# JBanks/GraphGym

Measured on AMD Instinct MI355X. Metric: aggregated edges/sec + achieved HBM GB/s, GCN d=256 on 100M-edge scale-free, higher is better.
Workload: dtype f32

## Files before the change

### graphgym_amd/csrc/gemm.hip

```cpp
#include "common.h"
#include "vecio.h"
#include "bf16x3.h"
#include <limits.h>

namespace mp {

constexpr int BM = 128, BN = 128, BK = 16;

constexpr int kPlaneBytes = 16 * 256;
__device__ __forceinline__ int swz_off(int row, int ch) {
  return 256 * row + 16 * (ch ^ (((row & 3) << 2) | ((row >> 2) & 3)));
}
__device__ __forceinline__ bf16x8 tr_read8(const unsigned char* plane, int col0, int lane) {
  const int g = lane >> 4, q = (lane & 15) >> 2, p = lane & 3;
  const int chunk = ((col0 + 16 * (g & 1)) >> 3) + (p >> 1);
  const int r0 = 8 * (g >> 1) + q;
  typedef __attribute__((address_space(3))) s16x4 lds_s16x4;
  const s16x4 lo = __builtin_amdgcn_ds_read_tr16_b64_v4i16(
      (lds_s16x4*)(plane + swz_off(r0, chunk) + 8 * (p & 1)));
  const s16x4 hi = __builtin_amdgcn_ds_read_tr16_b64_v4i16(
      (lds_s16x4*)(plane + swz_off(r0 + 4, chunk) + 8 * (p & 1)));
  const s16x8 v = {lo[0], lo[1], lo[2], lo[3], hi[0], hi[1], hi[2], hi[3]};
  return __builtin_bit_cast(bf16x8, v);
}
#define MP_STASH8(IMG, AT, lo, hi)                                                                      \
  do {                                                                                                  \
    bf16x8 s_[3];                                                                                       \
    const float v_[8] = {lo[0], lo[1], lo[2], lo[3], hi[0], hi[1], hi[2], hi[3]};                       \
    split3_bf16(v_, s_[0], s_[1], s_[2]);                                                               \
    _Pragma("unroll") for (int pl_ = 0; pl_ < 3; ++pl_) *reinterpret_cast<bf16x8*>(&IMG[pl_] AT) = s_[pl_]; \
  } while (0)
#define MP_ZERO_ACC(acc, NI, NJ)                         \
  _Pragma("unroll") for (int i_ = 0; i_ < (NI); ++i_)    \
  _Pragma("unroll") for (int j_ = 0; j_ < (NJ); ++j_)    \
  _Pragma("unroll") for (int r_ = 0; r_ < 16; ++r_) acc[i_][j_][r_] = 0.f

template <bool DUAL, bool VEC>
__global__ __launch_bounds__(kBlock, 3) void dense_fused_kernel(const float* __restrict__ P, int64_t ldp,
                                                                const float* __restrict__ W,
                                                                const float* __restrict__ Q, int64_t ldq,
                                                                const float* __restrict__ Wid,
                                                                const float* __restrict__ bias, int act,
                                                                float* __restrict__ out, int64_t ldo, int64_t M,
                                                                int32_t F, int32_t d) {
  __shared__ __attribute__((aligned(16))) unsigned char Aimg[2][3][BM * 32];
  __shared__ __attribute__((aligned(16))) unsigned char Bimg[2][3][kPlaneBytes];
  const int tid = threadIdx.x;
  const int lane = tid & 63;
  const int wave = tid >> 6;
  const int wm = wave >> 1, wn = wave & 1;
  const int ncb = (d + BN - 1) / BN;
  const int64_t m0 = (int64_t)(blockIdx.x / ncb) * BM;
  const int n0 = (int)(blockIdx.x % ncb) * BN;

  const int a_row = tid >> 1;
  const int a_k = (tid & 1) * 8;
  const int b_k = tid >> 4;
  const int b_n = (tid & 15) * 8;
  const int64_t g_row = m0 + a_row;
  const bool row_ok = g_row < M;
  const int KT = DUAL ? 2 * F : F;

  f32x4 ra[2], rb[2];
  auto fetch = [&](int kt) {
    const f32x4 z = {0.f, 0.f, 0.f, 0.f};
    const int k = kt + a_k;
    const int kb = kt + b_k;
    if constexpr (VEC) {
      const bool second = DUAL && k >= F;
      const float* src = second ? Q + g_row * ldq + (k - F) : P + g_row * ldp + k;
      const bool ok = row_ok && k < KT;
      ra[0] = ok ? *reinterpret_cast<const f32x4*>(src) : z;
      ra[1] = ok ? *reinterpret_cast<const f32x4*>(src + 4) : z;
      const bool second_b = DUAL && kb >= F;
      const float* wsrc = (second_b ? Wid + (int64_t)(kb - F) * d : W + (int64_t)kb * d) + n0 + b_n;
#pragma unroll
      for (int q = 0; q < 2; ++q)
        rb[q] = (kb < KT && n0 + b_n + 4 * q < d) ? *reinterpret_cast<const f32x4*>(wsrc + 4 * q) : z;
    } else {
#pragma unroll
      for (int i = 0; i < 8; ++i) {
        const int ki = k + i;
        float v = 0.f;
        if (row_ok && ki < KT) v = (DUAL && ki >= F) ? Q[g_row * ldq + (ki - F)] : P[g_row * ldp + ki];
        ra[i >> 2][i & 3] = v;
      }
      const bool second_b = DUAL && kb >= F;
      const float* wrow = second_b ? Wid + (int64_t)(kb - F) * d : W + (int64_t)kb * d;
#pragma unroll
      for (int q = 0; q < 2; ++q)
#pragma unroll
        for (int i = 0; i < 4; ++i) {
          const int nn = n0 + b_n + 4 * q + i;
          rb[q][i] = (kb < KT && nn < d) ? wrow[nn] : 0.f;
        }
    }
  };
  auto stash = [&](int buf) {
    MP_STASH8(Aimg[buf], [a_row * 32 + (a_k >> 3) * 16], ra[0], ra[1]);
    MP_STASH8(Bimg[buf], [swz_off(b_k, b_n >> 3)], rb[0], rb[1]);
  };

  f32x16 acc[2][2];
  MP_ZERO_ACC(acc, 2, 2);

  fetch(0);
  stash(0);
  __syncthreads();
  const int ntiles = (KT + BK - 1) / BK;
  const int fr = lane & 31, fk = lane >> 5;
  for (int t = 0; t < ntiles; ++t) {
    const int buf = t & 1;
    if (t + 1 < ntiles) fetch((t + 1) * BK);
    {
      bf16x8 as[2][3], bs3[2][3];
#pragma unroll
      for (int i = 0; i < 2; ++i)
#pragma unroll
        for (int pl = 0; pl < 3; ++pl)
          as[i][pl] = *reinterpret_cast<const bf16x8*>(&Aimg[buf][pl][(wm * 64 + i * 32 + fr) * 32 + fk * 16]);
#pragma unroll
      for (int j = 0; j < 2; ++j)
#pragma unroll
        for (int pl = 0; pl < 3; ++pl) bs3[j][pl] = tr_read8(Bimg[buf][pl], wn * 64 + j * 32, lane);
#pragma unroll
      for (int i = 0; i < 2; ++i)
#pragma unroll
        for (int j = 0; j < 2; ++j) mfma6(acc[i][j], as[i], bs3[j]);
    }
    if (t + 1 < ntiles) stash(buf ^ 1);
    __syncthreads();
  }

#pragma unroll
  for (int j = 0; j < 2; ++j) {
    const int col = n0 + wn * 64 + j * 32 + fr;
    const bool col_ok = col < d;
    const float bv = (bias != nullptr && col_ok) ? bias[col] : 0.f;
#pragma unroll
    for (int i = 0; i < 2; ++i) {
#pragma unroll
      for (int r = 0; r < 16; ++r) {
        const int64_t row = m0 + wm * 64 + i * 32 + (r & 3) + 8 * (r >> 2) + 4 * fk;
        float v = acc[i][j][r] + bv;
        if (act == MP_ACT_RELU) v = fmaxf(v, 0.f);
        if (col_ok && row < M) out[row * ldo + col] = v;
      }
    }
  }
}


struct ChunkRows { int64_t mb, me; };
__device__ __forceinline__ ChunkRows chunk_rows(int64_t c, int64_t chunk, int64_t M) {
  const int64_t mb = c * chunk;
  return {mb, mb + chunk < M ? mb + chunk : M};
}

template <bool VEC, bool RELU>
__global__ __launch_bounds__(kBlock, 3) void dense_wgrad_kernel(const float* __restrict__ P, int64_t ldp,
                                                                const float* G, int64_t ldg,
                                                                const float* __restrict__ Y, int64_t ldy,
                                                                float* GM, int64_t ldgm,
                                                                int64_t M, int32_t F, int32_t d, int64_t chunk,
                                                                float* __restrict__ slabs,
                                                                float* __restrict__ bias_slabs) {
  constexpr int BT = 128;
  __shared__ __attribute__((aligned(16))) unsigned char Pimg[2][3][kPlaneBytes];
  __shared__ __attribute__((aligned(16))) unsigned char Gimg[2][3][kPlaneBytes];
  const int tid = threadIdx.x, lane = tid & 63, wave = tid >> 6;
  const int wm = wave >> 1, wn = wave & 1;
  const int tf = (F + BT - 1) / BT, td = (d + BT - 1) / BT;
  const int tile = blockIdx.x % (tf * td);
  const int64_t c = blockIdx.x / (tf * td);
  const int f0 = (tile / td) * BT, d0 = (tile % td) * BT;
  const ChunkRows cr = chunk_rows(c, chunk, M);
  const int64_t mb = cr.mb, me = cr.me;

  const int l_row = tid >> 4;
  const int l_col = (tid & 15) * 8;
  f32x4 rp[2], rg[2];
  const f32x4 z = {0.f, 0.f, 0.f, 0.f};
  auto fetch = [&](int64_t m0) {
    const int64_t m = m0 + l_row;
    const bool ok = m < me;
    const float* ps = P + m * ldp + f0 + l_col;
    const float* gs = G + m * ldg + d0 + l_col;
    if constexpr (VEC) {
      rp[0] = (ok && f0 + l_col < F) ? *reinterpret_cast<const f32x4*>(ps) : z;
      rp[1] = (ok && f0 + l_col + 4 < F) ? *reinterpret_cast<const f32x4*>(ps + 4) : z;
      rg[0] = (ok && d0 + l_col < d) ? *reinterpret_cast<const f32x4*>(gs) : z;
      rg[1] = (ok && d0 + l_col + 4 < d) ? *reinterpret_cast<const f32x4*>(gs + 4) : z;
      if constexpr (RELU) {
        const float* ys = Y + m * ldy + d0 + l_col;
        const f32x4 y0 = (ok && d0 + l_col < d) ? *reinterpret_cast<const f32x4*>(ys) : z;
        const f32x4 y1 = (ok && d0 + l_col + 4 < d) ? *reinterpret_cast<const f32x4*>(ys + 4) : z;
#pragma unroll
        for (int i = 0; i < 4; ++i) {
          rg[0][i] = y0[i] > 0.f ? rg[0][i] : 0.f;
          rg[1][i] = y1[i] > 0.f ? rg[1][i] : 0.f;
        }
        if (GM != nullptr && f0 == 0 && ok) {
          float* go = GM + m * ldgm + d0 + l_col;
          if (d0 + l_col < d) *reinterpret_cast<f32x4*>(go) = rg[0];
          if (d0 + l_col + 4 < d) *reinterpret_cast<f32x4*>(go + 4) = rg[1];
        }
      }
    } else {
#pragma unroll
      for (int i = 0; i < 8; ++i) {
        rp[i >> 2][i & 3] = (ok && f0 + l_col + i < F) ? ps[i] : 0.f;
        float gv = (ok && d0 + l_col + i < d) ? gs[i] : 0.f;
        if constexpr (RELU) {
          const bool in = ok && d0 + l_col + i < d;
          const float yv = in ? Y[m * ldy + d0 + l_col + i] : 0.f;
          gv = yv > 0.f ? gv : 0.f;
          if (GM != nullptr && f0 == 0 && in) GM[m * ldgm + d0 + l_col + i] = gv;
        }
        rg[i >> 2][i & 3] = gv;
      }
    }
  };
  auto stash = [&](int buf) {
    const float pv[8] = {rp[0][0], rp[0][1], rp[0][2], rp[0][3], rp[1][0], rp[1][1], rp[1][2], rp[1][3]};
    const float gv[8] = {rg[0][0], rg[0][1], rg[0][2], rg[0][3], rg[1][0], rg[1][1], rg[1][2], rg[1][3]};
    bf16x8 sp[3], sg[3];
    split3_bf16(pv, sp[0], sp[1], sp[2]);
    split3_bf16(gv, sg[0], sg[1], sg[2]);
    const int off = swz_off(l_row, l_col >> 3);
#pragma unroll
    for (int pl = 0; pl < 3; ++pl) {
      *reinterpret_cast<bf16x8*>(&Pimg[buf][pl][off]) = sp[pl];
      *reinterpret_cast<bf16x8*>(&Gimg[buf][pl][off]) = sg[pl];
    }
  };
  f32x16 acc[2][2];
  MP_ZERO_ACC(acc, 2, 2);

  const bool do_bias = bias_slabs != nullptr && f0 == 0;
  float bs[8];
#pragma unroll
  for (int i = 0; i < 8; ++i) bs[i] = 0.f;
  auto tally = [&]() {
#pragma unroll
    for (int i = 0; i < 4; ++i) { bs[i] += rg[0][i]; bs[4 + i] += rg[1][i]; }
  };

  const int fr = lane & 31, fk = lane >> 5;
  const int64_t ntiles = (me - mb + BK - 1) / BK;
  if (ntiles > 0) {
    fetch(mb);
    if (do_bias) tally();
    stash(0);
  }
  __syncthreads();
  for (int64_t t = 0; t < ntiles; ++t) {
    const int buf = (int)(t & 1);
    if (t + 1 < ntiles) {
      fetch(mb + (t + 1) * BK);
      if (do_bias) tally();
    }
    {
      bf16x8 as[2][3], bs3[2][3];
#pragma unroll
      for (int i = 0; i < 2; ++i)
#pragma unroll
        for (int pl = 0; pl < 3; ++pl) {
          as[i][pl] = tr_read8(Pimg[buf][pl], wm * 64 + i * 32, lane);
          bs3[i][pl] = tr_read8(Gimg[buf][pl], wn * 64 + i * 32, lane);
        }
#pragma unroll
      for (int i = 0; i < 2; ++i)
#pragma unroll
        for (int j = 0; j < 2; ++j) mfma6(acc[i][j], as[i], bs3[j]);
    }
    if (t + 1 < ntiles) stash(buf ^ 1);
    __syncthreads();
  }
  float* slab = slabs + c * (int64_t)F * d;
#pragma unroll
  for (int j = 0; j < 2; ++j) {
    const int col = d0 + wn * 64 + j * 32 + fr;
#pragma unroll
    for (int i = 0; i < 2; ++i) {
#pragma unroll
      for (int r = 0; r < 16; ++r) {
        const int row = f0 + wm * 64 + i * 32 + (r & 3) + 8 * (r >> 2) + 4 * fk;
        if (row < F && col < d) slab[(int64_t)row * d + col] = acc[i][j][r];
      }
    }
  }
  if (do_bias) {
    float (*red)[BT] = reinterpret_cast<float (*)[BT]>(&Pimg[0][0][0]);
    *reinterpret_cast<f32x4*>(&red[l_row][l_col]) = f32x4{bs[0], bs[1], bs[2], bs[3]};
    *reinterpret_cast<f32x4*>(&red[l_row][l_col + 4]) = f32x4{bs[4], bs[5], bs[6], bs[7]};
    __syncthreads();
    if (tid < BT && d0 + tid < d) {
      float sacc = 0.f;
#pragma unroll
      for (int r = 0; r < BK; ++r) sacc += red[r][tid];
      bias_slabs[c * (int64_t)d + d0 + tid] = sacc;
    }
  }
}

template <bool RELU>
__global__ __launch_bounds__(kBlock, 2) void dense_wgrad_wide_kernel(const float* __restrict__ P, int64_t ldp,
                                                                     const float* G, int64_t ldg,
                                                                     const float* __restrict__ Y, int64_t ldy,
                                                                     float* GM, int64_t ldgm,
                                                                     int64_t M, int32_t F, int32_t d, int64_t chunk,
                                                                     float* __restrict__ slabs,
                                                                     float* __restrict__ bias_slabs) {
  constexpr int BF = 256, BD = 128;
  __shared__ __attribute__((aligned(16))) unsigned char Pimg[2][3][2][kPlaneBytes];
  __shared__ __attribute__((aligned(16))) unsigned char Gimg[2][3][kPlaneBytes];
  const int tid = threadIdx.x, lane = tid & 63, wave = tid >> 6;
  const int tf = (F + BF - 1) / BF, td = (d + BD - 1) / BD;
  const int tile = blockIdx.x % (tf * td);
  const int64_t c = blockIdx.x / (tf * td);
  const int f0 = (tile / td) * BF, d0 = (tile % td) * BD;
  const ChunkRows cr = chunk_rows(c, chunk, M);
  const int64_t mb = cr.mb, me = cr.me;

  const int l_row = tid >> 4;
  const int l_col = (tid & 15) * 8;
  f32x4 rp[2][2], rg[2];
  const f32x4 z = {0.f, 0.f, 0.f, 0.f};
  auto fetch = [&](int64_t m0) {
    const int64_t m = m0 + l_row;
    const bool ok = m < me;
    const float* gs = G + m * ldg + d0 + l_col;
#pragma unroll
    for (int h = 0; h < 2; ++h) {
      const int fc = f0 + 128 * h + l_col;
      const float* ps = P + m * ldp + fc;
      rp[h][0] = (ok && fc < F) ? *reinterpret_cast<const f32x4*>(ps) : z;
      rp[h][1] = (ok && fc + 4 < F) ? *reinterpret_cast<const f32x4*>(ps + 4) : z;
    }
    rg[0] = (ok && d0 + l_col < d) ? *reinterpret_cast<const f32x4*>(gs) : z;
    rg[1] = (ok && d0 + l_col + 4 < d) ? *reinterpret_cast<const f32x4*>(gs + 4) : z;
    if constexpr (RELU) {
      const float* ys = Y + m * ldy + d0 + l_col;
      const f32x4 y0 = (ok && d0 + l_col < d) ? *reinterpret_cast<const f32x4*>(ys) : z;
      const f32x4 y1 = (ok && d0 + l_col + 4 < d) ? *reinterpret_cast<const f32x4*>(ys + 4) : z;
#pragma unroll
      for (int i = 0; i < 4; ++i) {
        rg[0][i] = y0[i] > 0.f ? rg[0][i] : 0.f;
        rg[1][i] = y1[i] > 0.f ? rg[1][i] : 0.f;
      }
      if (GM != nullptr && f0 == 0 && ok) {
        float* go = GM + m * ldgm + d0 + l_col;
        if (d0 + l_col < d) *reinterpret_cast<f32x4*>(go) = rg[0];
        if (d0 + l_col + 4 < d) *reinterpret_cast<f32x4*>(go + 4) = rg[1];
      }
    }
  };
  auto stash = [&](int buf) {
    const int off = swz_off(l_row, l_col >> 3);
#pragma unroll
    for (int h = 0; h < 2; ++h) {
      MP_STASH8(Pimg[buf], [h][off], rp[h][0], rp[h][1]);
    }
    MP_STASH8(Gimg[buf], [off], rg[0], rg[1]);
  };
  f32x16 acc[2][4];
  MP_ZERO_ACC(acc, 2, 4);

  const bool do_bias = bias_slabs != nullptr && f0 == 0;
  float bs[8];
#pragma unroll
  for (int i = 0; i < 8; ++i) bs[i] = 0.f;
  auto tally = [&]() {
#pragma unroll
    for (int i = 0; i < 4; ++i) { bs[i] += rg[0][i]; bs[4 + i] += rg[1][i]; }
  };

  const int fr = lane & 31, fk = lane >> 5;
  const int64_t ntiles = (me - mb + BK - 1) / BK;
  if (ntiles > 0) {
    fetch(mb);
    if (do_bias) tally();
    stash(0);
  }
  __syncthreads();
  for (int64_t t = 0; t < ntiles; ++t) {
    const int buf = (int)(t & 1);
    if (t + 1 < ntiles) {
      fetch(mb + (t + 1) * BK);
      if (do_bias) tally();
    }
    {
      bf16x8 as[2][3];
#pragma unroll
      for (int i = 0; i < 2; ++i)
#pragma unroll
        for (int pl = 0; pl < 3; ++pl) as[i][pl] = tr_read8(Pimg[buf][pl][wave >> 1], (wave & 1) * 64 + i * 32, lane);
#pragma unroll
      for (int j = 0; j < 4; ++j) {
        bf16x8 b3[3];
#pragma unroll
        for (int pl = 0; pl < 3; ++pl) b3[pl] = tr_read8(Gimg[buf][pl], j * 32, lane);
#pragma unroll
        for (int i = 0; i < 2; ++i) mfma6(acc[i][j], as[i], b3);
      }
    }
    if (t + 1 < ntiles) stash(buf ^ 1);
    __syncthreads();
  }
  float* slab = slabs + c * (int64_t)F * d;
#pragma unroll
  for (int j = 0; j < 4; ++j) {
    const int col = d0 + j * 32 + fr;
#pragma unroll
    for (int i = 0; i < 2; ++i) {
#pragma unroll
      for (int r = 0; r < 16; ++r) {
        const int row = f0 + wave * 64 + i * 32 + (r & 3) + 8 * (r >> 2) + 4 * fk;
        if (row < F && col < d) slab[(int64_t)row * d + col] = acc[i][j][r];
      }
    }
  }
  if (do_bias) {
    float (*red)[BD] = reinterpret_cast<float (*)[BD]>(&Pimg[0][0][0][0]);
    *reinterpret_cast<f32x4*>(&red[l_row][l_col]) = f32x4{bs[0], bs[1], bs[2], bs[3]};
    *reinterpret_cast<f32x4*>(&red[l_row][l_col + 4]) = f32x4{bs[4], bs[5], bs[6], bs[7]};
    __syncthreads();
    if (tid < BD && d0 + tid < d) {
      float sacc = 0.f;
#pragma unroll
      for (int r = 0; r < BK; ++r) sacc += red[r][tid];
      bias_slabs[c * (int64_t)d + d0 + tid] = sacc;
    }
  }
}

constexpr int WPC_MFMA_WAVES = 8, WPC_LOAD_WAVES = 4;
constexpr int WPC_THREADS = 64 * (WPC_MFMA_WAVES + WPC_LOAD_WAVES);

template <bool RELU, int DT>
__global__ __launch_bounds__(WPC_THREADS, 3) void dense_wgrad_pc_kernel(const float* __restrict__ P, int64_t ldp,
                                                                        const float* G, int64_t ldg,
                                                                        const float* __restrict__ Y, int64_t ldy,
                                                                        float* GM, int64_t ldgm, int64_t M, int32_t F,
                                                                        int32_t d, int64_t chunk,
                                                                        float* __restrict__ slabs,
                                                                        float* __restrict__ bias_slabs) {
  __shared__ __attribute__((aligned(16))) unsigned char Pimg[2][3][2][kPlaneBytes];
  __shared__ __attribute__((aligned(16))) unsigned char Gimg[2][3][DT][kPlaneBytes];
  const int tid = threadIdx.x, lane = tid & 63;
  const int wave = __builtin_amdgcn_readfirstlane(tid >> 6);
  const int tf = (F + 255) / 256, td = (d + 128 * DT - 1) / (128 * DT);
  const int tile = (int)(blockIdx.x % (unsigned)(tf * td));
  const int64_t c = blockIdx.x / (unsigned)(tf * td);
  const int f0 = (tile / td) * 256, d0 = (tile % td) * 128 * DT;
  const ChunkRows cr = chunk_rows(c, chunk, M);
  const int64_t mb = cr.mb, me = cr.me;
  const int64_t ntiles = (me - mb + BK - 1) / BK;

  constexpr int NSET = RELU ? 2 : 3;
  const int64_t nsteps = (ntiles + NSET - 1) / NSET * NSET;
  if (wave >= WPC_MFMA_WAVES) {
    const int lt = tid - 64 * WPC_MFMA_WAVES;
    const int l_row = lt >> 4;
    const int l_col = (lt & 15) * 8;
    const bool do_bias = bias_slabs != nullptr && f0 == 0;
    float bs[2][8];
#pragma unroll
    for (int h = 0; h < 2; ++h)
#pragma unroll
      for (int i = 0; i < 8; ++i) bs[h][i] = 0.f;
    bool pin[2], gin[2];
    int pcol[2], gcol[2];
#pragma unroll
    for (int h = 0; h < 2; ++h) {
      const int fc = 128 * h + l_col;
      pin[h] = f0 + fc < F; gin[h] = d0 + fc < d;
      pcol[h] = pin[h] ? f0 + fc : 0; gcol[h] = gin[h] ? d0 + fc : 0;
    }
    f32x4 rp[NSET][2][2], rg[NSET][2][2], ry[RELU ? NSET : 1][2][2];
    auto fetch = [&](int s, int64_t tile) {
      int64_t m = mb + tile * BK + l_row;
      m = m < me ? m : me - 1;
#pragma unroll
      for (int h = 0; h < 2; ++h) {
        const float* ps = P + m * ldp + pcol[h];
        rp[s][h][0] = *reinterpret_cast<const f32x4*>(ps);
        rp[s][h][1] = *reinterpret_cast<const f32x4*>(ps + 4);
        if (h < DT) {
          const float* gs = G + m * ldg + gcol[h];
          rg[s][h][0] = *reinterpret_cast<const f32x4*>(gs);
          rg[s][h][1] = *reinterpret_cast<const f32x4*>(gs + 4);
          if constexpr (RELU) {
            const float* ys = Y + m * ldy + gcol[h];
            ry[s][h][0] = *reinterpret_cast<const f32x4*>(ys);
            ry[s][h][1] = *reinterpret_cast<const f32x4*>(ys + 4);
          }
        }
      }
    };
    auto stash = [&](int s, int64_t tile, int buf) {
      const int off = swz_off(l_row, l_col >> 3);
      const int64_t m = mb + tile * BK + l_row;
      const bool ok = m < me;
#pragma unroll
      for (int h = 0; h < 2; ++h) {
        float pv[8];
#pragma unroll
        for (int i = 0; i < 8; ++i) pv[i] = (ok && pin[h]) ? rp[s][h][i >> 2][i & 3] : 0.f;
        bf16x8 sp[3];
        split3_bf16(pv, sp[0], sp[1], sp[2]);
#pragma unroll
        for (int pl = 0; pl < 3; ++pl) *reinterpret_cast<bf16x8*>(&Pimg[buf][pl][h][off]) = sp[pl];
        if (h < DT) {
          float gv[8];
#pragma unroll
          for (int i = 0; i < 8; ++i) {
            gv[i] = (ok && gin[h]) ? rg[s][h][i >> 2][i & 3] : 0.f;
            if constexpr (RELU) gv[i] = ry[s][h][i >> 2][i & 3] > 0.f ? gv[i] : 0.f;
          }
          if constexpr (RELU) {
            if (GM != nullptr && f0 == 0 && ok && gin[h]) {
              float* go = GM + m * ldgm + gcol[h];
              *reinterpret_cast<f32x4*>(go) = f32x4{gv[0], gv[1], gv[2], gv[3]};
              *reinterpret_cast<f32x4*>(go + 4) = f32x4{gv[4], gv[5], gv[6], gv[7]};
            }
          }
          bf16x8 sg[3];
          split3_bf16(gv, sg[0], sg[1], sg[2]);
#pragma unroll
          for (int pl = 0; pl < 3; ++pl) *reinterpret_cast<bf16x8*>(&Gimg[buf][pl][h][off]) = sg[pl];
          if (do_bias) {
#pragma unroll
            for (int i = 0; i < 8; ++i) bs[h][i] += gv[i];
          }
        }
      }
    };
#pragma unroll
    for (int k = 0; k < NSET; ++k) fetch(k, k);
    stash(0, 0, 0);
    fetch(0, NSET);
    role_barrier();
    for (int64_t base = 0; base < nsteps; base += NSET) {
#pragma unroll
      for (int u = 0; u < NSET; ++u) {
        const int64_t t = base + u;
        const int sidx = (u + 1) % NSET;
        stash(sidx, t + 1, (int)((t + 1) & 1));
        fetch(sidx, t + 1 + NSET);
        role_barrier();
      }
    }
    if (do_bias) {
      float (*red)[256] = reinterpret_cast<float (*)[256]>(&Pimg[0][0][0][0]);
#pragma unroll
      for (int h = 0; h < DT; ++h) {
        *reinterpret_cast<f32x4*>(&red[l_row][128 * h + l_col]) = f32x4{bs[h][0], bs[h][1], bs[h][2], bs[h][3]};
        *reinterpret_cast<f32x4*>(&red[l_row][128 * h + l_col + 4]) = f32x4{bs[h][4], bs[h][5], bs[h][6], bs[h][7]};
      }
    }
    role_barrier();
    if (do_bias && lt < 128 * DT && d0 + lt < d) {
      const float (*red)[256] = reinterpret_cast<const float (*)[256]>(&Pimg[0][0][0][0]);
      float sacc = 0.f;
#pragma unroll
      for (int r = 0; r < BK; ++r) sacc += red[r][lt];
      bias_slabs[c * (int64_t)d + d0 + lt] = sacc;
    }
  } else {
    constexpr int NI = DT;
    const int wf = DT == 2 ? wave >> 1 : wave;
    const int wd = DT == 2 ? wave & 1 : 0;
    const int f_lo = DT == 2 ? wf * 64 : wf * 32;
    const int fr = lane & 31, fk = lane >> 5;
    f32x16 acc[NI][4];
    MP_ZERO_ACC(acc, NI, 4);
    role_barrier();
    for (int64_t t = 0; t < nsteps; ++t) {
      const int buf = (int)(t & 1);
#pragma unroll
      for (int i = 0; i < NI; ++i) {
        bf16x8 as[3];
#pragma unroll
        for (int pl = 0; pl < 3; ++pl) as[pl] = tr_read8(Pimg[buf][pl][f_lo >> 7], (f_lo & 127) + i * 32, lane);
#pragma unroll
        for (int j = 0; j < 4; ++j) {
          bf16x8 b3[3];
#pragma unroll
          for (int pl = 0; pl < 3; ++pl) b3[pl] = tr_read8(Gimg[buf][pl][wd], j * 32, lane);
          mfma6(acc[i][j], as, b3);
          __builtin_amdgcn_sched_barrier(0);
        }
      }
      role_barrier();
    }
    role_barrier();
    float* slab = slabs + c * (int64_t)F * d;
#pragma unroll
    for (int j = 0; j < 4; ++j) {
      const int col = d0 + wd * 128 + j * 32 + fr;
#pragma unroll
      for (int i = 0; i < NI; ++i) {
#pragma unroll
        for (int r = 0; r < 16; ++r) {
          const int row = f0 + f_lo + i * 32 + (r & 3) + 8 * (r >> 2) + 4 * fk;
          if (row < F && col < d) slab[(int64_t)row * d + col] = acc[i][j][r];
        }
      }
    }
  }
}

template <bool RELU>
__global__ __launch_bounds__(kBlock) void narrow_wgrad_kernel(const float* __restrict__ P, int64_t ldp,
                                                              const float* G, int64_t ldg,
                                                              const float* __restrict__ Y, int64_t ldy, float* GM,
                                                              int64_t ldgm, int64_t M, int32_t F, int32_t d,
                                                              int64_t chunk, float* __restrict__ slabs,
                                                              float* __restrict__ bias_slabs) {
  const int c = blockIdx.y * kBlock + threadIdx.x;
  const int64_t ch = blockIdx.x;
  const ChunkRows cr = chunk_rows(ch, chunk, M);
  const int64_t mb = cr.mb, me = cr.me;
  if (c >= d) return;
  float acc[8];
#pragma unroll
  for (int f = 0; f < 8; ++f) acc[f] = 0.f;
  float bs = 0.f;
  constexpr int UR = 4;
  for (int64_t m0 = mb; m0 < me; m0 += UR) {
    float gv[UR];
#pragma unroll
    for (int u = 0; u < UR; ++u) {
      const int64_t m = m0 + u;
      float v = 0.f;
      if (m < me) {
        v = G[m * ldg + c];
        if constexpr (RELU) {
          v = Y[m * ldy + c] > 0.f ? v : 0.f;
          if (GM != nullptr) GM[m * ldgm + c] = v;
        }
      }
      gv[u] = v;
    }
#pragma unroll
    for (int u = 0; u < UR; ++u) {
      const int64_t m = m0 + u;
      if (m < me) {
        bs += gv[u];
        const float* pr = P + m * ldp;
#pragma unroll
        for (int f = 0; f < 8; ++f)
          if (f < F) acc[f] = fmaf(pr[f], gv[u], acc[f]);
      }
    }
  }
  float* slab = slabs + ch * (int64_t)F * d;
  for (int f = 0; f < F; ++f) slab[(int64_t)f * d + c] = acc[f];
  if (bias_slabs != nullptr) bias_slabs[ch * (int64_t)d + c] = bs;
}

template <bool RELU, int FT>
__global__ __launch_bounds__(kBlock) void narrow_wgrad_vec_kernel(const float* __restrict__ P, int64_t ldp,
                                                                  const float* G, int64_t ldg,
                                                                  const float* __restrict__ Y, int64_t ldy, float* GM,
                                                                  int64_t ldgm, int64_t M, int32_t F, int32_t d,
                                                                  int64_t chunk, float* __restrict__ slabs,
                                                                  float* __restrict__ bias_slabs) {
  __shared__ __attribute__((aligned(16))) float red[kBlock * 4 * (FT + 1)];
  const int ncg = d >> 2;
  const int nrl = kBlock / ncg;
  const int cg = threadIdx.x % ncg, rl = threadIdx.x / ncg;
  const int64_t ch = blockIdx.x;
  const ChunkRows cr = chunk_rows(ch, chunk, M);
  const int64_t mb = cr.mb, me = cr.me;
  f32x4 acc[FT];
#pragma unroll
  for (int f = 0; f < FT; ++f) acc[f] = f32x4{0.f, 0.f, 0.f, 0.f};
  f32x4 bs = {0.f, 0.f, 0.f, 0.f};
  constexpr int UR = FT == 1 ? 8 : 4;
  for (int64_t m0 = mb + rl; m0 < me; m0 += (int64_t)UR * nrl) {
    f32x4 gv[UR], yv[UR];
    float pv[UR][FT];
#pragma unroll
    for (int u = 0; u < UR; ++u) {
      int64_t m = m0 + (int64_t)u * nrl;
      m = m < me ? m : me - 1;
      gv[u] = *reinterpret_cast<const f32x4*>(G + m * ldg + 4 * cg);
      if constexpr (RELU) yv[u] = *reinterpret_cast<const f32x4*>(Y + m * ldy + 4 * cg);
      const float* pr = P + m * ldp;
#pragma unroll
      for (int f = 0; f < FT; ++f) pv[u][f] = pr[f < F ? f : F - 1];
    }
#pragma unroll
    for (int u = 0; u < UR; ++u) {
      const int64_t m = m0 + (int64_t)u * nrl;
      if (m < me) {
        f32x4 v = gv[u];
        if constexpr (RELU) {
          v[0] = yv[u][0] > 0.f ? v[0] : 0.f; v[1] = yv[u][1] > 0.f ? v[1] : 0.f;
          v[2] = yv[u][2] > 0.f ? v[2] : 0.f; v[3] = yv[u][3] > 0.f ? v[3] : 0.f;
          if (GM != nullptr) *reinterpret_cast<f32x4*>(GM + m * ldgm + 4 * cg) = v;
        }
        bs += v;
#pragma unroll
        for (int f = 0; f < FT; ++f) acc[f] += pv[u][f] * v;
      }
    }
  }
#pragma unroll
  for (int f = 0; f < FT; ++f) *reinterpret_cast<f32x4*>(&red[((rl * (FT + 1) + f) * ncg + cg) * 4]) = acc[f];
  *reinterpret_cast<f32x4*>(&red[((rl * (FT + 1) + FT) * ncg + cg) * 4]) = bs;
  __syncthreads();
  if (rl == 0) {
    float* slab = slabs + ch * (int64_t)F * d;
    for (int f = 0; f <= FT; ++f) {
      if (f < F || (f == FT && bias_slabs != nullptr)) {
        f32x4 t = {0.f, 0.f, 0.f, 0.f};
        for (int r = 0; r < nrl; ++r) t += *reinterpret_cast<const f32x4*>(&red[((r * (FT + 1) + f) * ncg + cg) * 4]);
        if (f < FT) *reinterpret_cast<f32x4*>(slab + (int64_t)f * d + 4 * cg) = t;
        else *reinterpret_cast<f32x4*>(bias_slabs + ch * (int64_t)d + 4 * cg) = t;
      }
    }
  }
}

__global__ __launch_bounds__(kBlock) void narrow_out_wgrad_kernel(const float* __restrict__ P, int64_t ldp,
                                                                  const float* __restrict__ G, int64_t ldg, int64_t M,
                                                                  int32_t F, int32_t d, int64_t chunk,
                                                                  float* __restrict__ slabs,
                                                                  float* __restrict__ bias_slabs) {
  __shared__ float red[64][4][17];
  const int ncg = F >> 2;
  const int64_t ch = blockIdx.x;
  const ChunkRows cr = chunk_rows(ch, chunk, M);
  const int64_t mb = cr.mb, me = cr.me;
  float* slab = slabs + ch * (int64_t)F * d;
  for (int cg0 = 0; cg0 < ncg; cg0 += 64) {
    const int ng = ncg - cg0 < 64 ? ncg - cg0 : 64;
    const int nrl = kBlock / 64;
    const int cgi = threadIdx.x & 63, rl = threadIdx.x >> 6;
    const bool on = cgi < ng;
    const int f0 = 4 * (cg0 + cgi);
    float acc[4][16];
#pragma unroll
    for (int f = 0; f < 4; ++f)
#pragma unroll
      for (int j = 0; j < 16; ++j) acc[f][j] = 0.f;
    float bs[16];
#pragma unroll
    for (int j = 0; j < 16; ++j) bs[j] = 0.f;
    constexpr int UR = 4;
    for (int64_t m0 = mb + rl; m0 < me; m0 += (int64_t)UR * nrl) {
      f32x4 pv[UR];
      float gv[UR][16];
#pragma unroll
      for (int u = 0; u < UR; ++u) {
        int64_t m = m0 + (int64_t)u * nrl;
        m = m < me ? m : me - 1;
        pv[u] = on ? *reinterpret_cast<const f32x4*>(P + m * ldp + f0) : f32x4{0.f, 0.f, 0.f, 0.f};
#pragma unroll
        for (int j = 0; j < 16; ++j) gv[u][j] = G[m * ldg + (j < d ? j : d - 1)];
      }
#pragma unroll
      for (int u = 0; u < UR; ++u) {
        if (m0 + (int64_t)u * nrl < me) {
#pragma unroll
          for (int j = 0; j < 16; ++j) {
            bs[j] += gv[u][j];
#pragma unroll
            for (int f = 0; f < 4; ++f) acc[f][j] = fmaf(pv[u][f], gv[u][j], acc[f][j]);
          }
        }
      }
    }
    for (int r = 0; r < nrl; ++r) {
      if (rl == r && on) {
#pragma unroll
        for (int f = 0; f < 4; ++f)
#pragma unroll
          for (int j = 0; j < 16; ++j) red[cgi][f][j] = (r == 0 ? 0.f : red[cgi][f][j]) + acc[f][j];
      }
      __syncthreads();
    }
    if (rl == 0 && on) {
#pragma unroll
      for (int f = 0; f < 4; ++f)
        for (int j = 0; j < d; ++j) slab[(int64_t)(f0 + f) * d + j] = red[cgi][f][j];
    }
    __syncthreads();
    if (bias_slabs != nullptr && cg0 == 0) {
      for (int r = 0; r < nrl; ++r) {
        if (rl == r && cgi == 0) {
#pragma unroll
          for (int j = 0; j < 16; ++j) red[0][0][j] = (r == 0 ? 0.f : red[0][0][j]) + bs[j];
        }
        __syncthreads();
      }
      if (threadIdx.x < d) bias_slabs[ch * (int64_t)d + threadIdx.x] = red[0][0][threadIdx.x];
      __syncthreads();
    }
  }
}

__global__ __launch_bounds__(kBlock) void slab_reduce_kernel(const float* __restrict__ slabs, int64_t n_slab,
                                                             int64_t elems, float* __restrict__ out) {
  __shared__ float part[16][16];
  const int e = threadIdx.x & 15, sl = threadIdx.x >> 4;
  for (int64_t i0 = (int64_t)blockIdx.x * 16; i0 < elems; i0 += (int64_t)gridDim.x * 16) {
    const int64_t i = i0 + e;
    float a0 = 0.f, a1 = 0.f, a2 = 0.f, a3 = 0.f;
    if (i < elems) {
      int64_t c = sl;
      for (; c + 48 < n_slab; c += 64) {
        a0 += slabs[c * elems + i];
        a1 += slabs[(c + 16) * elems + i];
        a2 += slabs[(c + 32) * elems + i];
        a3 += slabs[(c + 48) * elems + i];
      }
      for (; c < n_slab; c += 16) a0 += slabs[c * elems + i];
    }
    part[sl][e] = (a0 + a1) + (a2 + a3);
    __syncthreads();
    if (sl == 0 && i < elems) {
      float acc = 0.f;
#pragma unroll
      for (int r = 0; r < 16; ++r) acc += part[r][e];
      out[i] = acc;
    }
    __syncthreads();
  }
}

static int64_t wgrad_chunk(int64_t M, int32_t F, int32_t d) {
  if (F <= 8) return 2048;
  if (d <= 16) return 4096;
  int64_t chunk = 4096;
  while (chunk < 65536 && ceil_div(M, chunk) > 1024) chunk *= 2;
  return chunk;
}

static bool al16(const void* p) { return p == nullptr || ((uintptr_t)p % 16) == 0; }

static int64_t wgrad_pc_chunk(int64_t M) {
  int64_t c = ceil_div(M, (int64_t)kNumCU);
  c = ceil_div(c, (int64_t)BK) * BK;
  return c < 4096 ? 4096 : c;
}

}

using namespace mp;

extern "C" {

int mp_dense_fused_f32(const float* P, int64_t ldp, const float* W, const float* Q, int64_t ldq,
                       const float* Wid, const float* bias, int act, float* out, int64_t ldo, int64_t M,
                       int32_t F, int32_t d, mp_stream_t stream) {
  if (M < 0 || F <= 0 || d <= 0 || !P || !W || !out || ldp < F || ldo < d) return MP_ERR_INVALID_ARG;
  if ((Q == nullptr) != (Wid == nullptr) || (Q && ldq < F)) return MP_ERR_INVALID_ARG;
  if (act != MP_ACT_NONE && act != MP_ACT_RELU) return MP_ERR_INVALID_ARG;
  if (M == 0) return MP_OK;
  const bool vec = !(F % 8 || d % 4 || ldp % 4 || (Q && ldq % 4)) && al16(P) && al16(W) && al16(Q) && al16(Wid);
  const int64_t nblocks = ceil_div(d, BN) * ceil_div(M, BM);
  if (nblocks >= INT32_MAX) return MP_ERR_UNSUPPORTED;
  dim3 grid((unsigned)nblocks);
  hipStream_t st = as_stream(stream);
  with_bools(Q != nullptr, vec, [&](auto dual, auto v) {
    hipLaunchKernelGGL((dense_fused_kernel<decltype(dual)::value, decltype(v)::value>), grid, dim3(kBlock), 0, st, P, ldp,
                       W, Q, ldq, Wid, bias, act, out, ldo, M, F, d);
  });
  MP_LAUNCH_CHECK();
  return MP_OK;
}

int mp_dense_wgrad_ws_bytes(int64_t M, int32_t F, int32_t d, size_t* bytes_host) {
  if (!bytes_host || M < 0 || F <= 0 || d <= 0) return MP_ERR_INVALID_ARG;
  *bytes_host = (size_t)ceil_div(M > 0 ? M : 1, wgrad_chunk(M, F, d)) * ((size_t)F * d + d) * 4;
  return MP_OK;
}

static int reduce_slabs(const void* ws, int64_t n_slab, int32_t F, int32_t d, float* dW, const float* bias_slabs,
                        float* dbias, hipStream_t st) {
  hipLaunchKernelGGL(slab_reduce_kernel, dim3(flat_grid((int64_t)F * d * 16)), dim3(kBlock), 0, st, (const float*)ws,
                     n_slab, (int64_t)F * d, dW);
  MP_LAUNCH_CHECK();
  if (dbias) {
    hipLaunchKernelGGL(slab_reduce_kernel, dim3(flat_grid((int64_t)d * 16)), dim3(kBlock), 0, st, bias_slabs, n_slab,
                       (int64_t)d, dbias);
    MP_LAUNCH_CHECK();
  }
  return MP_OK;
}

static int wgrad_common(const float* P, int64_t ldp, const float* G, int64_t ldg, const float* Y, int64_t ldy,
                        float* GM, int64_t ldgm, int64_t M, int32_t F, int32_t d, float* dW, float* dbias, void* ws,
                        size_t ws_bytes, hipStream_t st) {
  if (M < 0 || F <= 0 || d <= 0 || !dW || (M > 0 && (!P || !G)) || ldp < F || ldg < d) return MP_ERR_INVALID_ARG;
  if (Y && ldy < d) return MP_ERR_INVALID_ARG;
  if (GM && (!Y || ldgm < d)) return MP_ERR_INVALID_ARG;
  if (M == 0) {
    MP_HIP(hipMemsetAsync(dW, 0, (size_t)F * d * 4, st));
    if (dbias) MP_HIP(hipMemsetAsync(dbias, 0, (size_t)d * 4, st));
    return MP_OK;
  }
  const bool vec = !(F % 4 || d % 4 || ldp % 4 || ldg % 4 || (Y && ldy % 4) || (GM && ldgm % 4)) && al16(P) &&
                   al16(G) && al16(Y) && al16(GM);
  const int64_t chunk = wgrad_chunk(M, F, d);
  const int64_t n_chunk = ceil_div(M, chunk);
  const size_t need = (size_t)n_chunk * ((size_t)F * d + d) * 4;
  if (!ws || ws_bytes < need) return MP_ERR_WORKSPACE;
  float* bias_slabs = dbias ? (float*)ws + (size_t)n_chunk * F * d : nullptr;
  const int64_t tiles = ceil_div(F, 128) * ceil_div(d, 128);
  if (tiles * n_chunk >= INT32_MAX) return MP_ERR_UNSUPPORTED;
  if (F <= 8) {
    const dim3 ngrid((unsigned)n_chunk, (unsigned)ceil_div(d, kBlock));
    const bool nvec = d % 4 == 0 && d <= 4 * kBlock && kBlock % (d / 4) == 0 && ldg % 4 == 0 && al16(G) &&
                      (!Y || (ldy % 4 == 0 && al16(Y))) && (!GM || (ldgm % 4 == 0 && al16(GM))) &&
                      al16(ws) && (!bias_slabs || al16(bias_slabs));
    with_bools(Y != nullptr, F == 1, [&](auto relu, auto one) {
      constexpr bool R = decltype(relu)::value;
      if (nvec)
        hipLaunchKernelGGL((narrow_wgrad_vec_kernel<R, decltype(one)::value ? 1 : 8>), dim3((unsigned)n_chunk),
                           dim3(kBlock), 0, st, P, ldp, G, ldg, Y, ldy, GM, ldgm, M, F, d, chunk, (float*)ws, bias_slabs);
      else
        hipLaunchKernelGGL(narrow_wgrad_kernel<R>, ngrid, dim3(kBlock), 0, st, P, ldp, G, ldg, Y, ldy, GM, ldgm, M, F,
                           d, chunk, (float*)ws, bias_slabs);
    });
    MP_LAUNCH_CHECK();
    return reduce_slabs(ws, n_chunk, F, d, dW, bias_slabs, dbias, st);
  }
  if (!Y && d <= 16 && F % 4 == 0 && ldp % 4 == 0 && al16(P)) {
    hipLaunchKernelGGL(narrow_out_wgrad_kernel, dim3((unsigned)n_chunk), dim3(kBlock), 0, st, P, ldp, G, ldg, M, F, d,
                       chunk, (float*)ws, bias_slabs);
    MP_LAUNCH_CHECK();
    return reduce_slabs(ws, n_chunk, F, d, dW, bias_slabs, dbias, st);
  }
  if (vec && F > 128 && d >= 64 && F % 8 == 0 && d % 8 == 0) {
    const int64_t pc_chunk = wgrad_pc_chunk(M);
    const int64_t n_pc = ceil_div(M, pc_chunk);
    float* pc_bias = dbias ? (float*)ws + (size_t)n_pc * F * d : nullptr;
    const int64_t pc_tiles = ceil_div(F, 256) * ceil_div(d, d > 128 ? 256 : 128);
    if (n_pc * pc_tiles >= INT32_MAX) return MP_ERR_UNSUPPORTED;
    with_bools(Y != nullptr, d > 128, [&](auto relu, auto two) {
      hipLaunchKernelGGL((dense_wgrad_pc_kernel<decltype(relu)::value, decltype(two)::value ? 2 : 1>),
                         dim3((unsigned)(n_pc * pc_tiles)), dim3(WPC_THREADS), 0, st, P, ldp, G, ldg, Y, ldy, GM, ldgm, M,
                         F, d, pc_chunk, (float*)ws, pc_bias);
    });
    MP_LAUNCH_CHECK();
    return reduce_slabs(ws, n_pc, F, d, dW, pc_bias, dbias, st);
  }
  const bool wide = vec && F > 128;
  const int64_t wtiles = wide ? ceil_div(F, 256) * ceil_div(d, 128) : tiles;
  if (wtiles * n_chunk >= INT32_MAX) return MP_ERR_UNSUPPORTED;
  const dim3 grid((unsigned)(wtiles * n_chunk));
  with_bools(Y != nullptr, vec, [&](auto relu, auto v) {
    constexpr bool R = decltype(relu)::value;
    if (wide)
      hipLaunchKernelGGL(dense_wgrad_wide_kernel<R>, grid, dim3(kBlock), 0, st, P, ldp, G, ldg, Y, ldy, GM, ldgm, M, F, d,
                         chunk, (float*)ws, bias_slabs);
    else
      hipLaunchKernelGGL((dense_wgrad_kernel<decltype(v)::value, R>), grid, dim3(kBlock), 0, st, P, ldp, G, ldg, Y, ldy,
                         GM, ldgm, M, F, d, chunk, (float*)ws, bias_slabs);
  });
  MP_LAUNCH_CHECK();
  return reduce_slabs(ws, n_chunk, F, d, dW, bias_slabs, dbias, st);
}

int mp_dense_wgrad_f32(const float* P, int64_t ldp, const float* G, int64_t ldg, int64_t M, int32_t F,
                       int32_t d, float* dW, float* dbias, void* ws, size_t ws_bytes, mp_stream_t stream) {
  return wgrad_common(P, ldp, G, ldg, nullptr, 0, nullptr, 0, M, F, d, dW, dbias, ws, ws_bytes, as_stream(stream));
}

int mp_dense_wgrad_relu_f32(const float* P, int64_t ldp, const float* G, int64_t ldg, const float* Y, int64_t ldy,
                            float* GM, int64_t ldgm, int64_t M, int32_t F, int32_t d, float* dW, float* dbias,
                            void* ws, size_t ws_bytes, mp_stream_t stream) {
  if (!Y) return MP_ERR_INVALID_ARG;
  return wgrad_common(P, ldp, G, ldg, Y, ldy, GM, ldgm, M, F, d, dW, dbias, ws, ws_bytes, as_stream(stream));
}

}
```

Measured before the change: 6.131 billion.

## Restructure wgrad kernels: unpredicated prefetch, LDS-staged G, resized chunking

The MFMA weight-gradient kernel now issues unconditional clamped global loads and defers masking, ReLU gating, GM writes and bias tallies into the stash step. Sched barriers keep those loads in flight across the MFMA phase, and B-fragments are read per column to cut register pressure. The narrow-output wgrad kernel is templated on output width, stages G rows through double-buffered LDS and software-pipelines P loads. Chunk sizing for F<=128 now targets about three blocks per CU. The new code adds complexity and extra LDS use, and on the last tile it does redundant clamped loads.

```diff
diff --git a/graphgym_amd/csrc/gemm.hip b/graphgym_amd/csrc/gemm.hip
--- a/graphgym_amd/csrc/gemm.hip
+++ b/graphgym_amd/csrc/gemm.hip
@@ -179,51 +179,67 @@
 
   const int l_row = tid >> 4;
   const int l_col = (tid & 15) * 8;
-  f32x4 rp[2], rg[2];
-  const f32x4 z = {0.f, 0.f, 0.f, 0.f};
+  f32x4 rp[2], rg[2], ry[2];
+  const bool do_gm = RELU && GM != nullptr && f0 == 0;
+  const bool do_bias = bias_slabs != nullptr && f0 == 0;
+  float bs[8];
+#pragma unroll
+  for (int i = 0; i < 8; ++i) bs[i] = 0.f;
+  const int pc0 = f0 + l_col, gc0 = d0 + l_col;
   auto fetch = [&](int64_t m0) {
+    int64_t m = m0 + l_row;
+    m = m < me ? m : me - 1;
+    const float* ps = P + m * ldp;
+    const float* gs = G + m * ldg;
+    const float* ys = RELU ? Y + m * ldy : nullptr;
+    if constexpr (VEC) {
+#pragma unroll
+      for (int q = 0; q < 2; ++q) {
+        const int pc = pc0 + 4 * q < F ? pc0 + 4 * q : 0, gc = gc0 + 4 * q < d ? gc0 + 4 * q : 0;
+        rp[q] = *reinterpret_cast<const f32x4*>(ps + pc);
+        rg[q] = *reinterpret_cast<const f32x4*>(gs + gc);
+        if constexpr (RELU) ry[q] = *reinterpret_cast<const f32x4*>(ys + gc);
+      }
+    } else {
+      int pcv = pc0, gcv = gc0;
+      asm volatile("" : "+v"(pcv), "+v"(gcv));
+#pragma unroll
+      for (int i = 0; i < 8; ++i) {
+        const int pc = pcv + i < F ? pcv + i : 0, gc = gcv + i < d ? gcv + i : 0;
+        rp[i >> 2][i & 3] = ps[pc];
+        rg[i >> 2][i & 3] = gs[gc];
+        if constexpr (RELU) ry[i >> 2][i & 3] = ys[gc];
+      }
+    }
+  };
+  auto stash = [&](int buf, int64_t m0) {
     const int64_t m = m0 + l_row;
     const bool ok = m < me;
-    const float* ps = P + m * ldp + f0 + l_col;
-    const float* gs = G + m * ldg + d0 + l_col;
-    if constexpr (VEC) {
-      rp[0] = (ok && f0 + l_col < F) ? *reinterpret_cast<const f32x4*>(ps) : z;
-      rp[1] = (ok && f0 + l_col + 4 < F) ? *reinterpret_cast<const f32x4*>(ps + 4) : z;
-      rg[0] = (ok && d0 + l_col < d) ? *reinterpret_cast<const f32x4*>(gs) : z;
-      rg[1] = (ok && d0 + l_col + 4 < d) ? *reinterpret_cast<const f32x4*>(gs + 4) : z;
-      if constexpr (RELU) {
-        const float* ys = Y + m * ldy + d0 + l_col;
-        const f32x4 y0 = (ok && d0 + l_col < d) ? *reinterpret_cast<const f32x4*>(ys) : z;
-        const f32x4 y1 = (ok && d0 + l_col + 4 < d) ? *reinterpret_cast<const f32x4*>(ys + 4) : z;
-#pragma unroll
-        for (int i = 0; i < 4; ++i) {
-          rg[0][i] = y0[i] > 0.f ? rg[0][i] : 0.f;
-          rg[1][i] = y1[i] > 0.f ? rg[1][i] : 0.f;
+    float pv[8], gv[8];
+#pragma unroll
+    for (int i = 0; i < 8; ++i) {
+      const int e = VEC ? (i & 4) : i;
+      pv[i] = (ok && pc0 + e < F) ? rp[i >> 2][i & 3] : 0.f;
+      gv[i] = (ok && gc0 + e < d) ? rg[i >> 2][i & 3] : 0.f;
+      if constexpr (RELU) gv[i] = ry[i >> 2][i & 3] > 0.f ? gv[i] : 0.f;
+    }
+    if constexpr (RELU) {
+      if (do_gm && ok) {
+        float* go = GM + m * ldgm + gc0;
+        if constexpr (VEC) {
+          if (gc0 < d) *reinterpret_cast<f32x4*>(go) = f32x4{gv[0], gv[1], gv[2], gv[3]};
+          if (gc0 + 4 < d) *reinterpret_cast<f32x4*>(go + 4) = f32x4{gv[4], gv[5], gv[6], gv[7]};
+        } else {
+#pragma unroll
+          for (int i = 0; i < 8; ++i)
+            if (gc0 + i < d) go[i] = gv[i];
         }
-        if (GM != nullptr && f0 == 0 && ok) {
-          float* go = GM + m * ldgm + d0 + l_col;
-          if (d0 + l_col < d) *reinterpret_cast<f32x4*>(go) = rg[0];
-          if (d0 + l_col + 4 < d) *reinterpret_cast<f32x4*>(go + 4) = rg[1];
-        }
-      }
-    } else {
-#pragma unroll
-      for (int i = 0; i < 8; ++i) {
-        rp[i >> 2][i & 3] = (ok && f0 + l_col + i < F) ? ps[i] : 0.f;
-        float gv = (ok && d0 + l_col + i < d) ? gs[i] : 0.f;
-        if constexpr (RELU) {
-          const bool in = ok && d0 + l_col + i < d;
-          const float yv = in ? Y[m * ldy + d0 + l_col + i] : 0.f;
-          gv = yv > 0.f ? gv : 0.f;
-          if (GM != nullptr && f0 == 0 && in) GM[m * ldgm + d0 + l_col + i] = gv;
-        }
-        rg[i >> 2][i & 3] = gv;
-      }
-    }
-  };
-  auto stash = [&](int buf) {
-    const float pv[8] = {rp[0][0], rp[0][1], rp[0][2], rp[0][3], rp[1][0], rp[1][1], rp[1][2], rp[1][3]};
-    const float gv[8] = {rg[0][0], rg[0][1], rg[0][2], rg[0][3], rg[1][0], rg[1][1], rg[1][2], rg[1][3]};
+      }
+    }
+    if (do_bias) {
+#pragma unroll
+      for (int i = 0; i < 8; ++i) bs[i] += gv[i];
+    }
     bf16x8 sp[3], sg[3];
     split3_bf16(pv, sp[0], sp[1], sp[2]);
     split3_bf16(gv, sg[0], sg[1], sg[2]);
@@ -237,44 +253,33 @@
   f32x16 acc[2][2];
   MP_ZERO_ACC(acc, 2, 2);
 
-  const bool do_bias = bias_slabs != nullptr && f0 == 0;
-  float bs[8];
-#pragma unroll
-  for (int i = 0; i < 8; ++i) bs[i] = 0.f;
-  auto tally = [&]() {
-#pragma unroll
-    for (int i = 0; i < 4; ++i) { bs[i] += rg[0][i]; bs[4 + i] += rg[1][i]; }
-  };
-
   const int fr = lane & 31, fk = lane >> 5;
   const int64_t ntiles = (me - mb + BK - 1) / BK;
-  if (ntiles > 0) {
-    fetch(mb);
-    if (do_bias) tally();
-    stash(0);
-  }
+  fetch(mb);
+  stash(0, mb);
   __syncthreads();
   for (int64_t t = 0; t < ntiles; ++t) {
     const int buf = (int)(t & 1);
-    if (t + 1 < ntiles) {
-      fetch(mb + (t + 1) * BK);
-      if (do_bias) tally();
-    }
+    const int64_t mn = mb + (t + 1) * BK;
+    fetch(mn);
+    __builtin_amdgcn_sched_barrier(0);
     {
-      bf16x8 as[2][3], bs3[2][3];
+      bf16x8 as[2][3];
 #pragma unroll
       for (int i = 0; i < 2; ++i)
 #pragma unroll
-        for (int pl = 0; pl < 3; ++pl) {
-          as[i][pl] = tr_read8(Pimg[buf][pl], wm * 64 + i * 32, lane);
-          bs3[i][pl] = tr_read8(Gimg[buf][pl], wn * 64 + i * 32, lane);
-        }
-#pragma unroll
-      for (int i = 0; i < 2; ++i)
-#pragma unroll
-        for (int j = 0; j < 2; ++j) mfma6(acc[i][j], as[i], bs3[j]);
-    }
-    if (t + 1 < ntiles) stash(buf ^ 1);
+        for (int pl = 0; pl < 3; ++pl) as[i][pl] = tr_read8(Pimg[buf][pl], wm * 64 + i * 32, lane);
+#pragma unroll
+      for (int j = 0; j < 2; ++j) {
+        bf16x8 b3[3];
+#pragma unroll
+        for (int pl = 0; pl < 3; ++pl) b3[pl] = tr_read8(Gimg[buf][pl], wn * 64 + j * 32, lane);
+#pragma unroll
+        for (int i = 0; i < 2; ++i) mfma6(acc[i][j], as[i], b3);
+      }
+    }
+    __builtin_amdgcn_sched_barrier(0);
+    stash(buf ^ 1, mn);
     __syncthreads();
   }
   float* slab = slabs + c * (int64_t)F * d;
@@ -726,61 +731,106 @@
   }
 }
 
-__global__ __launch_bounds__(kBlock) void narrow_out_wgrad_kernel(const float* __restrict__ P, int64_t ldp,
-                                                                  const float* __restrict__ G, int64_t ldg, int64_t M,
-                                                                  int32_t F, int32_t d, int64_t chunk,
-                                                                  float* __restrict__ slabs,
-                                                                  float* __restrict__ bias_slabs) {
-  __shared__ float red[64][4][17];
+template <int DJ>
+__global__ __launch_bounds__(kBlock, DJ == 8 ? 3 : 2) void narrow_out_wgrad_kernel(const float* __restrict__ P, int64_t ldp,
+                                                                     const float* __restrict__ G, int64_t ldg,
+                                                                     int64_t M, int32_t F, int32_t d, int64_t chunk,
+                                                                     float* __restrict__ slabs,
+                                                                     float* __restrict__ bias_slabs) {
+  constexpr int UR = 4;
+  constexpr int SB = kBlock;
+  __shared__ __attribute__((aligned(16))) float gs[2][SB][DJ];
+  __shared__ float red[64][4][DJ + 1];
+  const int tid = threadIdx.x;
   const int ncg = F >> 2;
+  int cgs = 4;
+  while ((1 << cgs) < ncg && cgs < 6) ++cgs;
+  const int nrl = kBlock >> cgs;
+  const int cgi = tid & ((1 << cgs) - 1), rl = tid >> cgs;
   const int64_t ch = blockIdx.x;
   const ChunkRows cr = chunk_rows(ch, chunk, M);
   const int64_t mb = cr.mb, me = cr.me;
   float* slab = slabs + ch * (int64_t)F * d;
+  const int jb = (cgi & 15) < d ? (cgi & 15) : d - 1;
+  const int step = UR * nrl;
+  const int64_t nstage = (me - mb + SB - 1) / SB;
   for (int cg0 = 0; cg0 < ncg; cg0 += 64) {
     const int ng = ncg - cg0 < 64 ? ncg - cg0 : 64;
-    const int nrl = kBlock / 64;
-    const int cgi = threadIdx.x & 63, rl = threadIdx.x >> 6;
     const bool on = cgi < ng;
     const int f0 = 4 * (cg0 + cgi);
-    float acc[4][16];
+    const float* pcol = P + (on ? f0 : 0);
+    float acc[4][DJ];
 #pragma unroll
     for (int f = 0; f < 4; ++f)
 #pragma unroll
-      for (int j = 0; j < 16; ++j) acc[f][j] = 0.f;
-    float bs[16];
-#pragma unroll
-    for (int j = 0; j < 16; ++j) bs[j] = 0.f;
-    constexpr int UR = 4;
-    for (int64_t m0 = mb + rl; m0 < me; m0 += (int64_t)UR * nrl) {
-      f32x4 pv[UR];
-      float gv[UR][16];
+      for (int j = 0; j < DJ; ++j) acc[f][j] = 0.f;
+    float bsum = 0.f;
+    f32x4 pv[2][UR];
+    float gr[DJ];
+    auto load_g = [&](int64_t sb) {
+      int64_t m = mb + sb * SB + tid;
+      m = m < me ? m : me - 1;
+      int dv = d;
+      asm volatile("" : "+s"(dv));
+      const float* grow = G + m * ldg;
+#pragma unroll
+      for (int j = 0; j < DJ; ++j) gr[j] = grow[j < dv ? j : dv - 1];
+    };
+    auto store_g = [&](int buf) {
+#pragma unroll
+      for (int q = 0; q < DJ / 4; ++q)
+        *reinterpret_cast<f32x4*>(&gs[buf][tid][4 * q]) = f32x4{gr[4 * q], gr[4 * q + 1], gr[4 * q + 2], gr[4 * q + 3]};
+    };
+    auto load_p = [&](int s, int64_t m0) {
 #pragma unroll
       for (int u = 0; u < UR; ++u) {
         int64_t m = m0 + (int64_t)u * nrl;
         m = m < me ? m : me - 1;
-        pv[u] = on ? *reinterpret_cast<const f32x4*>(P + m * ldp + f0) : f32x4{0.f, 0.f, 0.f, 0.f};
-#pragma unroll
-        for (int j = 0; j < 16; ++j) gv[u][j] = G[m * ldg + (j < d ? j : d - 1)];
-      }
+        pv[s][u] = *reinterpret_cast<const f32x4*>(pcol + m * ldp);
+      }
+      __builtin_amdgcn_sched_barrier(0);
+    };
+    auto fma = [&](int s, int64_t m0, int buf, int lr0) {
 #pragma unroll
       for (int u = 0; u < UR; ++u) {
         if (m0 + (int64_t)u * nrl < me) {
-#pragma unroll
-          for (int j = 0; j < 16; ++j) {
-            bs[j] += gv[u][j];
-#pragma unroll
-            for (int f = 0; f < 4; ++f) acc[f][j] = fmaf(pv[u][f], gv[u][j], acc[f][j]);
+          const float* g = gs[buf][lr0 + u * nrl];
+          bsum += g[jb];
+#pragma unroll
+          for (int q = 0; q < DJ / 4; ++q) {
+            const f32x4 gq = *reinterpret_cast<const f32x4*>(g + 4 * q);
+#pragma unroll
+            for (int i = 0; i < 4; ++i)
+#pragma unroll
+              for (int f = 0; f < 4; ++f) acc[f][4 * q + i] = fmaf(pv[s][u][f], gq[i], acc[f][4 * q + i]);
           }
         }
       }
+    };
+    load_g(0);
+    store_g(0);
+    load_p(0, mb + rl);
+    __syncthreads();
+    for (int64_t sb = 0; sb < nstage; ++sb) {
+      const int buf = (int)(sb & 1);
+      const int64_t s0 = mb + sb * SB;
+      load_g(sb + 1);
+      for (int lr = rl; lr < SB && s0 + lr - rl < me; lr += 2 * step) {
+        const int64_t m0 = s0 + lr;
+        load_p(1, m0 + step);
+        fma(0, m0, buf, lr);
+        load_p(0, m0 + 2 * step);
+        fma(1, m0 + step, buf, lr + step);
+      }
+      store_g(buf ^ 1);
+      __syncthreads();
     }
     for (int r = 0; r < nrl; ++r) {
       if (rl == r && on) {
 #pragma unroll
         for (int f = 0; f < 4; ++f)
 #pragma unroll
-          for (int j = 0; j < 16; ++j) red[cgi][f][j] = (r == 0 ? 0.f : red[cgi][f][j]) + acc[f][j];
+          for (int j = 0; j < DJ; ++j) red[cgi][f][j] = (r == 0 ? 0.f : red[cgi][f][j]) + acc[f][j];
       }
       __syncthreads();
     }
@@ -792,13 +842,10 @@
     __syncthreads();
     if (bias_slabs != nullptr && cg0 == 0) {
       for (int r = 0; r < nrl; ++r) {
-        if (rl == r && cgi == 0) {
-#pragma unroll
-          for (int j = 0; j < 16; ++j) red[0][0][j] = (r == 0 ? 0.f : red[0][0][j]) + bs[j];
-        }
+        if (rl == r && cgi < d) red[0][0][cgi] = (r == 0 ? 0.f : red[0][0][cgi]) + bsum;
         __syncthreads();
       }
-      if (threadIdx.x < d) bias_slabs[ch * (int64_t)d + threadIdx.x] = red[0][0][threadIdx.x];
+      if (tid < d) bias_slabs[ch * (int64_t)d + tid] = red[0][0][tid];
       __syncthreads();
     }
   }
@@ -833,9 +880,16 @@
   }
 }
 
+constexpr int64_t kWgradSlots = 3 * kNumCU;
+
 static int64_t wgrad_chunk(int64_t M, int32_t F, int32_t d) {
   if (F <= 8) return 2048;
   if (d <= 16) return 4096;
+  if (F <= 128) {
+    const int64_t slots = kWgradSlots / ceil_div((int64_t)d, (int64_t)128);
+    const int64_t chunk = ceil_div(ceil_div(M, slots > 0 ? slots : 1), (int64_t)BK) * BK;
+    return chunk < 1024 ? 1024 : chunk;
+  }
   int64_t chunk = 4096;
   while (chunk < 65536 && ceil_div(M, chunk) > 1024) chunk *= 2;
   return chunk;
@@ -932,8 +986,12 @@
     return reduce_slabs(ws, n_chunk, F, d, dW, bias_slabs, dbias, st);
   }
   if (!Y && d <= 16 && F % 4 == 0 && ldp % 4 == 0 && al16(P)) {
-    hipLaunchKernelGGL(narrow_out_wgrad_kernel, dim3((unsigned)n_chunk), dim3(kBlock), 0, st, P, ldp, G, ldg, M, F, d,
-                       chunk, (float*)ws, bias_slabs);
+    if (d <= 8)
+      hipLaunchKernelGGL(narrow_out_wgrad_kernel<8>, dim3((unsigned)n_chunk), dim3(kBlock), 0, st, P, ldp, G, ldg, M, F,
+                         d, chunk, (float*)ws, bias_slabs);
+    else
+      hipLaunchKernelGGL(narrow_out_wgrad_kernel<16>, dim3((unsigned)n_chunk), dim3(kBlock), 0, st, P, ldp, G, ldg, M, F,
+                         d, chunk, (float*)ws, bias_slabs);
     MP_LAUNCH_CHECK();
     return reduce_slabs(ws, n_chunk, F, d, dW, bias_slabs, dbias, st);
   }
```

New measurement: 6.014 billion. -1.9%, worse.
